# jovoy/SolarAxionRayTracing

Hardware: AMD Instinct MI355X
Metric: rays/sec (higher is better)
Workload: dtype f64

## Files before the change

### solaraxionraytracing_amd/csrc/sart_api.hip

```cpp
#include <hip/hip_runtime.h>
#include <rccl/rccl.h>
#include <dlfcn.h>
#include <sys/mman.h>
#include <unistd.h>

#include <algorithm>
#include <atomic>
#include <cmath>
#include <condition_variable>
#include <thread>
#include <cstdio>
#include <cstdlib>
#include <cstring>
#include <limits>
#include <map>
#include <mutex>
#include <string>
#include <vector>

#include "../../include/sart.h"
#include "sart_device.h"

namespace sart {
void launch_trace_histogram(const HotA& H, const HotB& HB, const DevBlob* blob, const TraceArgs& A, double* acc, int n_blocks,
// ... 16 lines not shown
                               double* shared_row, int n_blocks, hipStream_t stream, bool fast, bool fixed);
int angular_scan_blocks_per_cu(bool fast);
void launch_ascan_images(const HotA& H, const HotB& HB, const DevBlob* blob, const TraceArgs& A, const AScanArgs& AN, double* img_partials,
                         double* rows, double* shared_row, int n_blocks, hipStream_t stream, bool fast, bool fixed);
int ascan_images_blocks_per_cu(bool fast);
int energy_scan_blocks_per_cu(bool rotated);
void launch_trace_energy_scan(const HotA& H, const HotB& HB, const DevBlob* blob, const TraceArgs& A, const EScanArgs& EN, double* rows,
                              double* shared_row, int n_blocks, hipStream_t stream, bool rotated, bool fixed);
int shell_histogram_blocks_per_cu(bool rotated);
void launch_shell_histogram(const HotA& H, const HotB& HB, const DevBlob* blob, const TraceArgs& A, double* acc, const ShellArgs& SH,
                            int n_blocks, hipStream_t stream, bool rotated, bool fixed);
void launch_finalize_shells(const void* in, double* out, int n_shells, int n_energies1, int spectra, double q_w, double q_w2,
                            void* check_dev, hipStream_t stream);
int channel_histogram_blocks_per_cu(bool rotated);
void launch_channel_histogram(const HotA& H, const HotB& HB, const DevBlob* blob, const TraceArgs& A, double* acc, const ChannelArgs& CH,
                              int n_blocks, hipStream_t stream, bool rotated, bool fixed);
void launch_finalize_channels(const void* in, double* out, int n_channels, int n_energies1, int spectra, size_t n_img, double q_w,
                              double q_w2, void* check_dev, hipStream_t stream);
void launch_channel_fractions(const double* rates_dev, const double* total_dev, double* frac_dev, int n_channels, int stride,
                              size_t n_cells, unsigned long long* first_bad_dev, hipStream_t stream);
int origin_histogram_blocks_per_cu(bool rotated);
void launch_origin_histogram(const HotA& H, const HotB& HB, const DevBlob* blob, const TraceArgs& A, double* acc, const OriginArgs& OG,
                             int n_blocks, hipStream_t stream, bool rotated, bool fixed);
void launch_finalize_origin(const void* in, double* out, size_t n_cells, double q_w, double q_w2, void* check_dev, hipStream_t stream);
int aperture_histogram_blocks_per_cu(bool rotated);
void launch_aperture_histogram(const HotA& H, const HotB& HB, const DevBlob* blob, const TraceArgs& A, double* acc, const ApertureArgs& AP,
                               int n_blocks, hipStream_t stream, bool rotated, bool fixed);
int histogram_block_of(int variant);
void launch_trace_records(const HotA& H, const HotB& HB, const DevBlob* blob, const TraceArgs& A, sart_axion_t* out, int n_blocks,
                          hipStream_t stream, const double* uniforms_dev);
void launch_mirror_miss_count(const HotA& H, const DevBlob* blob, const TraceArgs& A, unsigned long long* counts, int n_blocks, hipStream_t stream);
void launch_radial_verdicts(const HotA& H, const DevBlob* blob, const double* radii, int n, uint32_t* out_table, uint32_t* out_compares,
                            hipStream_t stream);
int records_block();
int compact_chunk_max();
void launch_compact_records(const sart_axion_t* rec, uint32_t n, sart_axion_t* out, unsigned long long capacity, uint32_t* block_counts,
                            unsigned long long* block_first, unsigned long long* counts, hipStream_t stream);
void launch_stage_columns(const HotA& H, const HotB& HB, const DevBlob* blob, const TraceArgs& A, uint64_t* stage, uint32_t* flags,
                          uint32_t mask, int n_blocks, hipStream_t stream);
void launch_compact_columns(const uint64_t* stage, const uint32_t* flags, uint32_t n, uint32_t mask, unsigned long long ray_id0, uint64_t* out,
                            unsigned long long capacity, uint32_t* block_counts, unsigned long long* block_first,
                            unsigned long long* counts, hipStream_t stream);
int histogram_blocks_per_cu(int variant);
void launch_build_solar_tables(const double* em_dev, const double* radii_dev, const double* energies_dev, int n_radii, int n_energies,
                               double* cdf_dev, double* row_sum_dev, double* rcdf_dev, uint16_t* rguide_dev, uint16_t* eguide_dev,
                               uint32_t* status_dev, hipStream_t stream);
void launch_cdf_hi32(const double* cdf_dev, uint32_t* out_dev, size_t n, hipStream_t stream);
}

using namespace sart;

namespace {

thread_local std::string g_err;
int fail(int code, const std::string& msg) {
  g_err = msg;
  return code;
}
#define SART_HIP(call)                                                                              \
  do {                                                                                              \
    hipError_t e_ = (call);                                                                         \
    if (e_ != hipSuccess)                                                                           \
      return fail(e_ == hipErrorOutOfMemory ? SART_ERR_OUT_OF_MEMORY : SART_ERR_NO_DEVICE,          \
                  std::string(#call) + ": " + hipGetErrorString(e_));                               \
  } while (0)

// ... 1421 lines not shown
}

int sart_get_radial_table(sart_context* c, double* breakpoints, uint32_t* verdicts, uint8_t* cells, int32_t* n_cells) {
  if (!c) return fail(SART_ERR_INVALID_ARGUMENT, "ctx is NULL");
  SART_HIP(hipSetDevice(c->device));
  if (int rc = refresh_derived(c)) return rc;
  if (int rc = sync_blob(c)) return rc;
  if (n_cells) *n_cells = c->params.lut_n;
  if (c->radial_n > 0) {
    const uint8_t* t = c->shell_lut.data() + kRadialTableOffset;
    if (breakpoints) std::memcpy(breakpoints, t + offsetof(RadialLds, b), static_cast<size_t>(c->radial_n) * sizeof(double));
    if (verdicts) std::memcpy(verdicts, t + offsetof(RadialLds, w), static_cast<size_t>(c->radial_n) * sizeof(uint32_t));
    if (cells) std::memcpy(cells, c->shell_lut.data() + kRadialCellsOffset, static_cast<size_t>(c->params.lut_n));
  }
  return c->radial_n;
}

__attribute__((visibility("default"))) int sart_internal_radial_verdicts(sart_context* c, const double* radii, int32_t n, uint32_t* by_table,
                                                                         uint32_t* by_compares) {
  if (!c || !radii || !by_table || !by_compares || n < 1) return fail(SART_ERR_INVALID_ARGUMENT, "invalid argument");
  SART_HIP(hipSetDevice(c->device));
  if (int rc = refresh_derived(c)) return rc;
  if (int rc = sync_blob(c)) return rc;
  if (!c->hot.radial_table) return fail(SART_ERR_UNSUPPORTED, "this setup has no radial verdict table");
  DevBuf<double> d_r;
  DevBuf<uint32_t> d_out;
  if (int rc = d_r.upload(radii, static_cast<size_t>(n))) return rc;
  if (int rc = d_out.resize(2 * static_cast<size_t>(n))) return rc;
  launch_radial_verdicts(c->hot, c->d_blob.p, d_r.p, n, d_out.p, d_out.p + n, c->stream);
  SART_HIP(hipGetLastError());
  SART_HIP(hipMemcpyAsync(by_table, d_out.p, static_cast<size_t>(n) * sizeof(uint32_t), hipMemcpyDeviceToHost, c->stream));
  SART_HIP(hipMemcpyAsync(by_compares, d_out.p + n, static_cast<size_t>(n) * sizeof(uint32_t), hipMemcpyDeviceToHost, c->stream));
  SART_HIP(hipStreamSynchronize(c->stream));
  return 0;
}

namespace {

class HostPrefault {
 public:
  HostPrefault(char* base, size_t bytes, size_t chunk_bytes, bool enabled, unsigned threads, bool keep = false)
      : base_(base), bytes_(bytes), chunk_(chunk_bytes), threads_(threads ? threads : 8u), keep_(keep) {
    n_chunks_ = (bytes + chunk_bytes - 1) / chunk_bytes;
    if (!enabled || bytes < (size_t(8) << 20)) { done_ = n_chunks_; return; }
    const long page = sysconf(_SC_PAGESIZE);
    page_ = page > 0 ? static_cast<size_t>(page) : 4096;
    const uintptr_t lo = (reinterpret_cast<uintptr_t>(base) + page_ - 1) / page_ * page_;
    const uintptr_t hi = (reinterpret_cast<uintptr_t>(base) + bytes) / page_ * page_;
    if (hi > lo) (void)madvise(reinterpret_cast<void*>(lo), hi - lo, MADV_HUGEPAGE);
    worker_ = std::thread([this] { run(); });
  }
  ~HostPrefault() {
    allow(0, true);
    if (worker_.joinable()) worker_.join();
  }
  void wait(size_t k) {
    allow(k + 1);
    std::unique_lock<std::mutex> lock(m_);
    cv_.wait(lock, [&] { return done_ > k; });
  }
  void set_lazy() { std::lock_guard<std::mutex> lock(m_); allowed_ = 0; }
  void allow(size_t chunks, bool stop = false) {
    {
      std::lock_guard<std::mutex> lock(m_);
      allowed_ = std::max(allowed_, std::min(chunks, n_chunks_));
      stop_ = stop_ || stop;
// ... 1859 lines not shown
```

### solaraxionraytracing_amd/csrc/sart_kernels.hip

```cpp
#include <hip/hip_runtime.h>
#include <stdint.h>
#include <string.h>

#include <type_traits>

#include "../../include/sart.h"
#include "sart_device.h"
#include "sart_math.h"

namespace sart {

struct U4 { uint32_t x, y, z, w; };
constexpr int kPhiloxRounds = 7;

__device__ __forceinline__ U4 philox4x32(uint32_t c0, uint32_t c1, uint32_t c2, uint32_t c3, uint32_t k0,
                                         uint32_t k1) {
#pragma unroll
  for (int r = 0; r < kPhiloxRounds; ++r) {
    const uint64_t p0 = (uint64_t)0xD2511F53u * c0;
    const uint64_t p1 = (uint64_t)0xCD9E8D57u * c2;
    const uint32_t hi0 = (uint32_t)(p0 >> 32), lo0 = (uint32_t)p0;
    const uint32_t hi1 = (uint32_t)(p1 >> 32), lo1 = (uint32_t)p1;
    const uint32_t n0 = __builtin_amdgcn_bitop3_b32(hi1, c1, k0, 0x96);
    const uint32_t n2 = __builtin_amdgcn_bitop3_b32(hi0, c3, k1, 0x96);
// ... 1136 lines not shown
#ifndef SART_PRIO_B
#define SART_PRIO_B 3
#endif
#ifndef SART_PRIO_ACC
#define SART_PRIO_ACC 1
#endif
constexpr int kQueue = 128;

struct __align__(16) TablesLds {
  double sincos[2 * kSinCosEntries];
  uint32_t rcdf_hi[kMaxRadii + 4];
  ShellDev shells[kMaxShells];
  uint16_t rguide[kRadiusGuideEntries + 6];
  uint8_t lut[kShellLutMax];
};

struct __align__(16) WaveRings {
  double X0[kQueue], Y0[kQueue], tsx[kQueue], tsy[kQueue];
  double path[kQueue], u5[kQueue];
  int idx[kQueue];
  uint32_t ray[kQueue];
  uint32_t u3hi[kQueue];
};
struct __align__(16) HistRings {
  double X0[kQueue], Y0[kQueue], tsx[kQueue], tsy[kQueue];
  double path[kQueue];
  uint2 cell[kQueue];
  uint32_t ray[kQueue];
  uint32_t u3hi[kQueue];
};
static_assert(sizeof(WaveRings) - sizeof(HistRings) == kQueue * sizeof(uint32_t) && sizeof(HistRings) % 512 == 0 &&
                  (kTileRingCells / kQueue * (sizeof(WaveRings) - sizeof(HistRings))) / sizeof(double) == kTileExtraCells + kRadialTableCells - kRingExtraCells,
              "what ring 1's packed cell frees is what the histogram kernels' image tile grows by");
template <int WAVES, typename Rings = WaveRings>
struct __align__(16) QueueLds {
  Rings w[WAVES];
};

template <int BLOCK>
__device__ __forceinline__ void stage_tables(TablesLds& S, const DevParams& P, const DevTables& T, bool radial_cells = false) {
  for (int i = threadIdx.x; i < 2 * kSinCosEntries; i += BLOCK) S.sincos[i] = as_global(T.sincos_tab)[i];
  for (int i = threadIdx.x; i < P.n_radii + 4; i += BLOCK) {
    const double c = (i < P.n_radii) ? as_global(T.flux_radius_cdf)[i] : 1.0;
    const unsigned long long t = __double2ull_rd(c * 4503599627370496.0) >> 20;
    S.rcdf_hi[i] = t > 0xFFFFFFFFull ? 0xFFFFFFFFu : (uint32_t)t;
  }
  for (int i = threadIdx.x; i < kRadiusGuideEntries; i += BLOCK) S.rguide[i] = as_global(T.radius_guide)[i];
  {
    const auto src = as_global(reinterpret_cast<const uint64_t*>(T.shells));
    uint64_t* dst = reinterpret_cast<uint64_t*>(S.shells);
    const int n = P.n_shells * (int)(sizeof(ShellDev) / 8);
    for (int i = threadIdx.x; i < n; i += BLOCK) dst[i] = src[i];
  }
  const uint8_t* lut = T.shell_lut + (radial_cells ? kRadialCellsOffset : 0);
  for (int i = threadIdx.x; i < P.lut_n; i += BLOCK) S.lut[i] = as_global(lut)[i];
  __syncthreads();
}

__device__ __forceinline__ void reload_hot(HotA& dst) {
  typedef const __attribute__((address_space(4))) uint32_t* kernarg_ptr;
  kernarg_ptr p = (kernarg_ptr)__builtin_amdgcn_kernarg_segment_ptr();
  asm volatile("" : "+s"(p));
  uint32_t* d = reinterpret_cast<uint32_t*>(&dst);
#pragma unroll
  for (int k = 0; k < (int)(sizeof(HotA) / 4); ++k) d[k] = p[k];
}

struct ZoneTable {
  int32_t n_zones;
  uint32_t zone_reached;
  uint32_t lo[kMaxZones], hi[kMaxZones];
};
static_assert(sizeof(ZoneTable) == sizeof(HotA) - offsetof(HotA, n_zones), "ZoneTable mirrors the tail of HotA");
static_assert(offsetof(WaveRings, u3hi) == offsetof(WaveRings, ray) + kQueue * sizeof(uint32_t) && offsetof(WaveRings, ray) % 8 == 0 &&
                  offsetof(HistRings, u3hi) == offsetof(HistRings, ray) + kQueue * sizeof(uint32_t) && offsetof(HistRings, ray) % 8 == 0,
              "the image tile uses ray + u3hi of every wave as 128 contiguous doubles");
__device__ __forceinline__ void reload_zones(ZoneTable& dst) {
  typedef const __attribute__((address_space(4))) uint32_t* kernarg_ptr;
  kernarg_ptr p = (kernarg_ptr)__builtin_amdgcn_kernarg_segment_ptr() + offsetof(HotA, n_zones) / 4;
  asm volatile("" : "+s"(p));
  uint32_t* d = reinterpret_cast<uint32_t*>(&dst);
#pragma unroll
  for (int k = 0; k < (int)(sizeof(ZoneTable) / 4); ++k) d[k] = p[k];
}

struct HistKernArgs {
  HotA H;
  const DevBlob* blob;
  TraceArgs A;
  double* acc;
  HotB HB;
  ScanArgs SC;
};
static_assert(offsetof(HistKernArgs, H) == 0 && offsetof(HistKernArgs, blob) == (sizeof(HotA) + 7) / 8 * 8 &&
                  offsetof(HistKernArgs, A) == offsetof(HistKernArgs, blob) + 8 &&
                  offsetof(HistKernArgs, acc) == offsetof(HistKernArgs, A) + sizeof(TraceArgs) &&
                  offsetof(HistKernArgs, HB) == offsetof(HistKernArgs, acc) + 8 &&
                  offsetof(HistKernArgs, SC) == offsetof(HistKernArgs, HB) + sizeof(HotB) && sizeof(HotA) % 4 == 0 &&
                  sizeof(TraceArgs) % 8 == 0 && sizeof(HotB) % 8 == 0,
              "reload_hot / reload_zones / reload_kernarg read the arguments at these offsets");
template <typename T>
__device__ __forceinline__ void reload_kernarg(T& dst, size_t byte_offset) {
  static_assert(sizeof(T) % 4 == 0, "dword granularity");
  typedef const __attribute__((address_space(4))) uint32_t* kernarg_ptr;
  kernarg_ptr p = (kernarg_ptr)__builtin_amdgcn_kernarg_segment_ptr() + byte_offset / 4;
  asm volatile("" : "+s"(p));
  uint32_t* d = reinterpret_cast<uint32_t*>(&dst);
#pragma unroll
  for (int k = 0; k < (int)(sizeof(T) / 4); ++k) d[k] = p[k];
}

template <int BLOCK, bool FAST, bool ROT, int GAS, bool PATHC, bool FIXED, bool SCAN = false>
__global__ __launch_bounds__(BLOCK) void trace_histogram_kernel(HotA H, const DevBlob* __restrict__ blob, TraceArgs A,
                                                                double* __restrict__ acc, HotB HBarg, ScanArgs SCarg) {
  constexpr bool BANDS = false;
#include "sart_trace_histogram.inc"
// ... 2260 lines not shown
__global__ __launch_bounds__(256) void radial_verdict_kernel(HotA H, const DevBlob* __restrict__ blob, const double* __restrict__ radii, int n,
                                                             uint32_t* __restrict__ out_table, uint32_t* __restrict__ out_compares) {
  struct Lds {
    TablesLds S;
    RadialLds R;
    double behind[kRadialMarked + 1 - kRadialMax];
    DevBlob B;
  };
  __shared__ Lds lds;
  {
    const uint64_t* src = reinterpret_cast<const uint64_t*>(blob);
    uint64_t* dst = reinterpret_cast<uint64_t*>(&lds.B);
    for (int i = threadIdx.x; i < (int)(sizeof(DevBlob) / 8); i += 256) dst[i] = src[i];
    for (int i = threadIdx.x; i < kRadialMarked + 1 - kRadialMax; i += 256) lds.behind[i] = 0.0;
    __syncthreads();
  }
  const DevParams& P = lds.B.P;
  {
    const auto src = as_global(reinterpret_cast<const uint64_t*>(lds.B.T.shell_lut + kRadialTableOffset));
    uint64_t* dst = reinterpret_cast<uint64_t*>(&lds.R);
    for (int i = threadIdx.x; i < kRadialTableCells; i += 256) dst[i] = src[i];
  }
  stage_tables<256>(lds.S, P, lds.B.T, true);
  const LdsTables L{lds.S.sincos, lds.S.rcdf_hi, lds.B.T.flux_radius_cdf, lds.S.rguide, lds.S.shells, lds.S.lut, &lds.R, &lds.B.T};
  const bool cand_on = H.telescope_kind != SART_TK_LLNL;
  const int i = blockIdx.x * 256 + threadIdx.x;
  if (i < n) {
    const double radial = radii[i];
    out_table[i] = radial_verdict_table(H, P, L, cand_on, radial);
    out_compares[i] = radial_verdict_compares(H, P, L.shells, lds.B.T.shell_lut, cand_on, radial);
  }
}

__global__ __launch_bounds__(kRecBlock) void mirror_miss_count_kernel(HotA H, const DevBlob* __restrict__ blob, TraceArgs A,
                                                                       unsigned long long* __restrict__ counts) {
  __shared__ TablesLds S;
  __shared__ DevBlob B;
  {
    const uint64_t* src = reinterpret_cast<const uint64_t*>(blob);
    uint64_t* dst = reinterpret_cast<uint64_t*>(&B);
    for (int i = threadIdx.x; i < (int)(sizeof(DevBlob) / 8); i += kRecBlock) dst[i] = src[i];
    __syncthreads();
  }
  const DevParams& P = B.P;
  stage_tables<kRecBlock>(S, P, B.T);
  const LdsTables L{S.sincos, S.rcdf_hi, B.T.flux_radius_cdf, S.rguide, S.shells, S.lut};
  uint32_t n[5] = {0, 0, 0, 0, 0};
  const uint64_t stride = (uint64_t)gridDim.x * kRecBlock;
  const uint64_t n_round = (A.n_rays + stride - 1) / stride * stride;
  for (uint64_t i = (uint64_t)blockIdx.x * kRecBlock + threadIdx.x; i < n_round; i += stride) {
    RayState st;
    bool sampled, reached;
    double radial;
    LaneMasks masks;
    double r3sq;
    const uint64_t ray_id = A.ray_id_offset + i;
    const uint32_t u3_hi = word_of(stream_block(ray_id >> 2, A.seed_lo, A.seed_hi), (uint32_t)ray_id & 3u);
    const bool alive = phase_a<false, -1, false, false, false>(H, P, L, A.seed_lo, A.seed_hi, ray_id, u3_hi, st, sampled, reached, radial, masks, nullptr, &r3sq) &&
                       i < A.n_rays;
    const ShellDev& sh = L.shells[st.shell];
    const double X0 = st.X0, Y0 = st.Y0, tsx = st.tsx, tsy = st.tsy;
    const double Q0 = fma(X0, X0, Y0 * Y0), D0 = fma(X0, tsx, Y0 * tsy), A0 = fma(tsx, tsx, tsy * tsy);
    double z1;
    uint64_t hit1_m;
    const bool hit1 = pick_root(A0 - sh.m1_k, D0 + sh.m1_hb, Q0 - sh.m1_cc, 0.0, sh.m1_zhi, z1, hit1_m);
    const double zcb = st.zcb;
// ... 611 lines not shown
  for (int k = 0; k < n_masses; ++k) { F.q_w[k] = q_w[k]; F.q_w2[k] = q_w2[k]; }
  hipLaunchKernelGGL(finalize_scan_kernel, dim3(1), dim3(64), 0, stream, reinterpret_cast<const long long*>(in), out, F, static_cast<FixedCheck*>(check_dev));
}
void launch_finalize_scan_bands(const void* rows, const void* shared_row, const void* in, double* out, const void* counts_in, double* counts_out,
                                int n_masses, int n_cells, const double* q_w, const double* q_w2, void* check_dev, hipStream_t stream) {
  FinalizeBandsArgs F;
  memset(&F, 0, sizeof F);
  F.n_masses = n_masses;
  F.n_cells = n_cells;
  for (int k = 0; k < n_masses; ++k) { F.q_w[k] = q_w[k]; F.q_w2[k] = q_w2[k]; }
  hipLaunchKernelGGL(finalize_scan_bands_kernel, dim3(n_masses + (counts_in ? 1 : 0)), dim3(64), 0, stream, static_cast<const long long*>(rows),
                     static_cast<const long long*>(shared_row), static_cast<const long long*>(in), out, static_cast<const long long*>(counts_in),
                     counts_out, F, static_cast<FixedCheck*>(check_dev));
}
int compact_chunk_max() { return kCompactBlock * kCompactMaxBlocks; }
void launch_compact_records(const sart_axion_t* rec, uint32_t n, sart_axion_t* out, unsigned long long capacity, uint32_t* block_counts,
                            unsigned long long* block_first, unsigned long long* counts, hipStream_t stream) {
  const uint32_t n_blocks = (n + kCompactBlock - 1) / kCompactBlock;
  hipLaunchKernelGGL(records_count_kernel, dim3(n_blocks), dim3(kCompactBlock), 0, stream, rec, n, block_counts, counts);
  hipLaunchKernelGGL(records_scan_kernel, dim3(1), dim3(kCompactMaxBlocks), 0, stream, block_counts, n_blocks, block_first, counts, n);
  hipLaunchKernelGGL(records_scatter_kernel, dim3(n_blocks), dim3(kCompactBlock), 0, stream, rec, n, block_first, out, capacity);
}
void launch_trace_records(const HotA& H, const HotB& HB, const DevBlob* blob, const TraceArgs& A, sart_axion_t* out, int n_blocks,
                          hipStream_t stream, const double* uniforms_dev) {
  hipLaunchKernelGGL(trace_records_kernel, dim3(n_blocks), dim3(kRecBlock), 0, stream, H, blob, A, out, HB, uniforms_dev);
}
void launch_mirror_miss_count(const HotA& H, const DevBlob* blob, const TraceArgs& A, unsigned long long* counts, int n_blocks, hipStream_t stream) {
  hipLaunchKernelGGL(mirror_miss_count_kernel, dim3(n_blocks), dim3(kRecBlock), 0, stream, H, blob, A, counts);
}
void launch_radial_verdicts(const HotA& H, const DevBlob* blob, const double* radii, int n, uint32_t* out_table, uint32_t* out_compares,
                            hipStream_t stream) {
  hipLaunchKernelGGL(radial_verdict_kernel, dim3((n + 255) / 256), dim3(256), 0, stream, H, blob, radii, n, out_table, out_compares);
}
void launch_stage_columns(const HotA& H, const HotB& HB, const DevBlob* blob, const TraceArgs& A, uint64_t* stage, uint32_t* flags,
                          uint32_t mask, int n_blocks, hipStream_t stream) {
  hipLaunchKernelGGL(columns_stage_kernel, dim3(n_blocks), dim3(kRecBlock), 0, stream, H, blob, A, stage, flags, HB, mask);
}
void launch_compact_columns(const uint64_t* stage, const uint32_t* flags, uint32_t n, uint32_t mask, unsigned long long ray_id0, uint64_t* out,
                            unsigned long long capacity, uint32_t* block_counts, unsigned long long* block_first,
                            unsigned long long* counts, hipStream_t stream) {
  const uint32_t n_blocks = (n + kCompactBlock - 1) / kCompactBlock;
  hipLaunchKernelGGL(columns_count_kernel, dim3(n_blocks), dim3(kCompactBlock), 0, stream, flags, n, block_counts, counts);
  hipLaunchKernelGGL(records_scan_kernel, dim3(1), dim3(kCompactMaxBlocks), 0, stream, block_counts, n_blocks, block_first, counts, n);
  hipLaunchKernelGGL(columns_scatter_kernel, dim3(n_blocks), dim3(kCompactBlock), 0, stream, stage, flags, n, block_first, out, capacity, mask,
                     ray_id0);
}

}
```

### solaraxionraytracing_amd/csrc/sart_trace_histogram.inc

```
  struct LdsLayout {
    TablesLds S;
    RadialLds R;
    double tile_extra[kTileExtraCells];
    DevBlob B;
    TraceArgs Ab;
    QueueLds<BLOCK / 64, HistRings> Q;
  };
  static_assert(sizeof(RadialLds) % 8 == 0 && (kRadialMarked + 1) * sizeof(double) <= sizeof(RadialLds) + kTileExtraCells * sizeof(double),
                "entry kRadialMarked of either column lies in the table or in the tile's cells");
  __shared__ LdsLayout lds;
  TablesLds& S = lds.S;
  QueueLds<BLOCK / 64, HistRings>& Q = lds.Q;
  static_assert(!PATHC || (FAST && !ROT && GAS >= 0), "the constant-path form belongs to the unrotated specialisations");
  static_assert(!SCAN || GAS != 0, "a mass scan needs the gas stage");
  static_assert(!SCAN || kScanMaxMasses * 2 * kScanLanes <= (BLOCK / 64) * kQueue, "the scan accumulators live in the image tile's 128 doubles per wave");
  __shared__ uint32_t scan_zero[kScanMaxMasses];
  static_assert(!BANDS || SCAN, "the bands belong to the mass scan");
  __shared__ uint32_t scan_band_n[BANDS ? kScanLanes : 1];
  static_assert((BLOCK / 64) * kQueue == kTileRingCells && kImageTileMax * kImageTileMax <= kTileRingCells + kTileExtraCells &&
                    kImageTileExtraMax * kImageTileExtraMax <= kTileExtraCells && BLOCK / 64 == kTileRingCells / kQueue,
                "the LDS image tile (host: kImageTileMax): 128 doubles per wave of this workgroup's rings + the cells behind the tables");
  static_assert((offsetof(LdsLayout, Q) % 512) == 0, "the rings are addressed with ds_*2st64 offsets (units of 512 bytes for 64-bit columns)");
  auto tile_cell_lo = [&](uint32_t t) -> double* {
    return PATHC ? &Q.w[t >> 7].path[t & 127u] : reinterpret_cast<double*>(&Q.w[t >> 7].ray[0]) + (t & 127u);
  };
  auto tile_cell = [&](uint32_t t) -> double* {
    return t < (uint32_t)kTileRingCells ? tile_cell_lo(t) : &lds.tile_extra[t - (uint32_t)kTileRingCells];
  };
  DevBlob& B = lds.B;
  TraceArgs& Ab = lds.Ab;
  {
    const uint64_t* src = reinterpret_cast<const uint64_t*>(blob);
    uint64_t* dst = reinterpret_cast<uint64_t*>(&B);
    for (int i = threadIdx.x; i < (int)(sizeof(DevBlob) / 8); i += BLOCK) dst[i] = src[i];
    if (threadIdx.x == 0) Ab = A;
    __syncthreads();
  }
  const DevParams& Pb = B.P;
  const DevTables& Tb = B.T;
  {
    uint64_t* q = reinterpret_cast<uint64_t*>(&Q);
    for (int i = threadIdx.x; i < (int)(sizeof(Q) / 8); i += BLOCK) q[i] = 0ull;
    for (int i = threadIdx.x; i < kTileExtraCells; i += BLOCK) lds.tile_extra[i] = 0.0;
    if (SCAN && threadIdx.x < kScanMaxMasses) scan_zero[threadIdx.x] = 0u;
    if (BANDS && threadIdx.x < kScanLanes) scan_band_n[threadIdx.x] = 0u;
  }
  constexpr bool RTAB = FAST;
  if (RTAB && H.radial_table) {
    const auto src = as_global(reinterpret_cast<const uint64_t*>(Tb.shell_lut + kRadialTableOffset));
    uint64_t* dst = reinterpret_cast<uint64_t*>(&lds.R);
    for (int i = threadIdx.x; i < kRadialTableCells; i += BLOCK) dst[i] = src[i];
  }
  stage_tables<BLOCK>(S, Pb, Tb, RTAB && H.radial_table);
  const LdsTables L{S.sincos, S.rcdf_hi, Tb.flux_radius_cdf, S.rguide, S.shells, S.lut, &lds.R, &Tb};

  const int lane = threadIdx.x & 63;
  const int wave = __builtin_amdgcn_readfirstlane((int)(threadIdx.x >> 6));
  const uint64_t waves_total = (uint64_t)gridDim.x * (BLOCK / 64);
  const uint64_t wave_global = (uint64_t)blockIdx.x * (BLOCK / 64) + wave;
  const bool early_reject = (SCAN && !PATHC) ? false : H.n_zones > 0;
  const uint64_t first_chunk = A.ray_id_offset >> 8;
  uint64_t id_base = first_chunk << 8;
  asm volatile("" : "+s"(id_base));
  const uint32_t rel_begin = (uint32_t)(A.ray_id_offset & 255u);
  const uint32_t rel_end = rel_begin + (uint32_t)A.n_rays;
  const uint32_t n_chunks = (rel_end + 255u) >> 8;

  uint32_t n_reached = 0, n_shell = 0, n_nickel = 0, n_till = 0, n_passed = 0;
  uint32_t n_outside = 0;
  using Sum = std::conditional_t<FIXED, long long, double>;
  Sum sum_w = 0, sum_w2 = 0, sum_x = 0, sum_y = 0, sum_r = 0;
  long long sum_wo = 0;
#ifdef SART_STAGE_TIMING
  uint64_t cyc_a0 = 0, cyc_a1 = 0, cyc_b = 0, cyc_bs[6] = {0, 0, 0, 0, 0, 0};
#endif
  uint32_t h0 = 0, t0 = 0;
// ... 21 lines not shown
    HotA Hl;
    reload_hot(Hl);
    constexpr bool ZEXT = FAST && !ROT && GAS >= 0;
    LaneMasks M;
    double r3sq = 0.0;
    (void)phase_a<FAST, ROT ? 1 : 0, ZEXT, PATHC, true, RTAB>(Hl, Pb, L, A.seed_lo, A.seed_hi, id_base + (uint64_t)rel, u3_hi, st, sampled, reached, radial,
                                                              M, HOLD_SINCOS ? &Ksc : nullptr, ROT ? nullptr : &r3sq);
    const uint64_t valid_m = ballot64(valid);
    n_reached += (uint32_t)__popcll(valid_m & M.reached);
    const uint64_t selected = valid_m & M.ok;
    n_shell += (uint32_t)__popcll(selected);
    uint64_t sure = 0ull;
    const uint64_t cand = (ROT || Hl.telescope_kind == SART_TK_LLNL) ? 0ull
                                                                     : (selected & (RTAB ? M.cand : ballot64(radial > (double)Pb.mirror_miss_radius)));
    if (cand) {
      if (RTAB && Hl.radial_table) r3sq = L.shells[st.shell].n1_r3sq;
      const double zl = Pb.l_mirror, xe = fma(zl, st.tsx, st.X0), ye = fma(zl, st.tsy, st.Y0);
      sure = cand & ballot64(fma(xe, xe, fma(ye, ye, kMirrorMissEps)) < r3sq) &
             ballot64(fma(st.tsx, st.tsx, st.tsy * st.tsy) < (double)Pb.mirror_miss_slope_sq);
      n_nickel += (uint32_t)__popcll(sure);
    }
#ifdef SART_DEBUG_KNOBS
    const uint64_t mask = (A.flags & 0x10000000u) ? 0ull : (selected & (RTAB ? M.keep : ~ballot64(radial < Pb.shell0_miss_radius)) & ~sure);
#else
    const uint64_t mask = selected & (RTAB ? M.keep : ~ballot64(radial < Pb.shell0_miss_radius)) & ~sure;
#endif
    const bool alive = __builtin_amdgcn_inverse_ballot_w64(mask);
    const uint32_t cnt = (uint32_t)__popcll(mask);
    if (alive) {
      asm volatile("; hot: ring 1 write");
      const uint32_t slot = prefix_from(mask, t1) % kQueue;
      Q.w[wave].X0[slot] = st.X0; Q.w[wave].Y0[slot] = st.Y0;
      Q.w[wave].tsx[slot] = st.tsx; Q.w[wave].tsy[slot] = st.tsy;
      if (!PATHC) Q.w[wave].path[slot] = st.path_cb;
      Q.w[wave].cell[slot] = make_uint2((uint32_t)(st.r_idx | (st.shell << 16)), st.u5_hi);
    }
    t1 += cnt;
    __builtin_amdgcn_s_setprio(0);
  };

  auto run_phase_b = [&](uint32_t n_valid) {
    SART_STAGE_MARK("B");
    __builtin_amdgcn_s_setprio(SART_PRIO_B);
    RayState st;
    const bool valid = (uint32_t)lane < n_valid;
    const uint32_t slot = (h1 + (uint32_t)lane) % kQueue;
    RayOut out;
    {
      st.X0 = Q.w[wave].X0[slot]; st.Y0 = Q.w[wave].Y0[slot];
      st.tsx = Q.w[wave].tsx[slot]; st.tsy = Q.w[wave].tsy[slot];
      st.path_cb = PATHC ? H.length_b : Q.w[wave].path[slot];
      const uint2 cell = Q.w[wave].cell[slot];
      st.u5 = u52(cell.y, 0u);
      st.u5_hi = cell.y;
      if (!ROT) {
        st.zcb = -(H.dz3 - H.dz1);
      } else {
        st.zcb = zcb_rotated(Pb.rx_s, -Pb.rx_c * Pb.ry_s, Pb.rx_c * Pb.ry_c, Pb.half_length_telescope, st.X0 + Pb.entrance_x,
                             st.Y0 + Pb.entrance_y, st.tsx, st.tsy, H.dz3 - H.dz1);
      }
      const int packed = (int)cell.x;
      st.r_idx = packed & 0xFFFF;
      st.shell = packed >> 16;
      const DevBlob& Bo = lds_opaque(B);
      HotB HB;
      reload_kernarg(HB, offsetof(HistKernArgs, HB));
      asm volatile("" :: "s"(HB.cdf_hi32), "s"(HB.energy_guide), "s"(HB.energy_tab), "s"(HB.refl), "s"(HB.refl_n_angles), "s"(HB.cdf_stride));
      phase_b<false, FAST, GAS, FAST && !ROT && GAS >= 0, SCAN>(Bo.P, L, HB, lds_opaque(Ab), st, (!FAST && H.test_active) ? Pb.n_energies : -1, valid, out, nullptr);
      if constexpr (SCAN) {
        SART_STAGE_MARK("SCAN");
        n_passed += (uint32_t)__popcll(out.m_passed);
        struct { int32_t n_masses, pad; } hdr;
        reload_kernarg(hdr, offsetof(HistKernArgs, SC));
        const uint32_t fl = (uint32_t)__builtin_amdgcn_readfirstlane((int)Ab.flags);
        const bool use_prob = !(fl & SART_CF_IGNORE_CONV_PROB) & ((GAS >= 0) ? (GAS == 1) : (__builtin_amdgcn_readfirstlane(Bo.P.stage_gas) != 0));
        const double term1 = Bo.P.gas_term1;
        const GasCos cos_lead = GasCos::make();
        uint32_t cell = 0u;
        if constexpr (BANDS) {
          struct { int32_t e0; uint32_t mul; } b0;
          struct { uint32_t window, unused; } b1;
          reload_kernarg(b0, offsetof(HistKernArgs, SC) + offsetof(ScanArgs, m) + offsetof(ScanMass, aux));
          reload_kernarg(b1, offsetof(HistKernArgs, SC) + offsetof(ScanArgs, m) + sizeof(ScanMass) + offsetof(ScanMass, aux));
          const uint32_t d = (uint32_t)(out.e_idx - b0.e0);
// ... 61 lines not shown
        sum_w2 = fma(out.weight, out.weight, sum_w2);
        sum_x += out.px;
        sum_y += out.py;
        sum_r += out.rdet;
      }
      const double fx = (out.px - Al.image_x_min) * Al.image_inv_step_x;
      const double fy = (out.py - Al.image_y_min) * Al.image_inv_step_y;
      const int nx = Al.image_nx, ny = Al.image_ny;
      const uint64_t inside_m = ballot64(fx >= 0.0) & ballot64(fx < (double)nx) & ballot64(fy >= 0.0) & ballot64(fy < (double)ny);
      const bool inside = __builtin_amdgcn_inverse_ballot_w64(inside_m);
      n_outside += inside ? 0u : 1u;
      if constexpr (FIXED) {
        if (out.m_passed & ~inside_m) {
          asm volatile("; rare: passed rays outside the image");
          sum_wo += inside ? 0ll : w_fx;
        }
      }
#ifdef SART_DEBUG_KNOBS
      const uint32_t rep_key = (Al.flags & 0x08000000u) ? blockIdx.x : (uint32_t)wave_global;
      double* const img = Al.replicas + (size_t)(rep_key & Al.replica_mask) * (size_t)Al.replica_stride;
#else
      double* const img = Al.replicas + (size_t)((uint32_t)wave_global & Al.replica_mask) * (size_t)Al.replica_stride;
#endif
#ifdef SART_DEBUG_KNOBS
      if (inside && !(Al.flags & 0x40000000u))
#else
      if (inside)
#endif
      {
        const uint32_t ix = (uint32_t)(int)fx, iy = (uint32_t)(int)fy;
        const uint32_t tn = (uint32_t)Al.tile_n;
        const uint32_t tx = ix - (uint32_t)Al.tile_x0, ty = iy - (uint32_t)Al.tile_y0;
        if ((tx < tn) & (ty < tn)) {
          const uint32_t t = ty * tn + tx + (uint32_t)Al.tile_base;
          if constexpr (FIXED)
            __hip_atomic_fetch_add(reinterpret_cast<unsigned long long*>(tile_cell(t)), (unsigned long long)w_fx, __ATOMIC_RELAXED,
                                   __HIP_MEMORY_SCOPE_WORKGROUP);
          else
            __hip_atomic_fetch_add(tile_cell(t), out.weight, __ATOMIC_RELAXED, __HIP_MEMORY_SCOPE_WORKGROUP);
        } else {
          const uint32_t pix = iy * (uint32_t)nx + ix;
          typedef __attribute__((address_space(1))) char* gbytes;
          if constexpr (FIXED) atomic_add_slot_i64((double*)((gbytes)img + pix * 8u), w_fx);
          else unsafeAtomicAdd((double*)((gbytes)img + pix * 8u), out.weight);
        }
      }
      if (Al.spectra) {
        double* rad = acc + (size_t)nx * (size_t)ny + SART_ACC_COUNT;
        double* en = rad + 2 * (size_t)Al.n_radial_bins;
        const size_t ne1 = (size_t)Pb.n_energies + 1;
        const int rb = min((int)(out.rdet * Al.radial_inv_bin), Al.n_radial_bins - 1);
        if constexpr (FIXED) {
          atomic_add_slot_i64(&rad[rb], 1);
          atomic_add_slot_i64(&rad[(size_t)Al.n_radial_bins + rb], w_fx);
          atomic_add_slot_i64(&en[out.e_idx], 1);
          atomic_add_slot_i64(&en[ne1 + out.e_idx], w_fx);
          atomic_add_slot_i64(&en[2 * ne1 + out.e_idx], to_fixed(out.reflect, kFixedReflectScale));
        } else {
          unsafeAtomicAdd(&rad[rb], 1.0);
          unsafeAtomicAdd(&rad[(size_t)Al.n_radial_bins + rb], out.weight);
          unsafeAtomicAdd(&en[out.e_idx], 1.0);
          unsafeAtomicAdd(&en[ne1 + out.e_idx], out.weight);
          unsafeAtomicAdd(&en[2 * ne1 + out.e_idx], out.reflect);
        }
      }
    }
    __builtin_amdgcn_s_setprio(0);
  };

  constexpr bool kZonesInVgprs = FAST;
  uint32_t zone_lo_v[kMaxZones], zone_hi_v[kMaxZones];
#pragma unroll
  for (int z = 0; z < kMaxZones; ++z) {
    zone_lo_v[z] = H.zone_lo[z];
    zone_hi_v[z] = H.zone_hi[z];
    if (kZonesInVgprs) asm volatile("" : "+v"(zone_lo_v[z]), "+v"(zone_hi_v[z]));
  }
  uint32_t zone_reached_v = H.zone_reached;
  if (kZonesInVgprs) asm volatile("" : "+v"(zone_reached_v));
  uint32_t chunk = (uint32_t)wave_global;
  const uint32_t lane4 = 4u * (uint32_t)lane;
  uint32_t pass = 0;
  U4 stream = U4{0u, 0u, 0u, 0u};
#ifdef SART_STAGE_TIMING
  const uint64_t cyc_start = __builtin_readcyclecounter();
  const uint64_t real_start = __builtin_amdgcn_s_memrealtime();
#define SART_STAMP(var) const uint64_t var = __builtin_readcyclecounter()
#define SART_SPAN(acc, t_begin) acc += __builtin_readcyclecounter() - (t_begin)
#else
#define SART_STAMP(var)
#define SART_SPAN(acc, t_begin)
#endif
  for (;;) {
    const bool have_new = chunk < n_chunks;
    SART_STAGE_MARK("LOOP");
    if (have_new) {
      SART_STAGE_MARK("A0");
      SART_STAMP(ts_a0);
      if (pass == 0u) {
        asm volatile("; hot x0.25: one block of the shared word stream per four passes");
        stream = stream_block(((first_chunk + (uint64_t)chunk) << 6) + (uint64_t)lane, A.seed_lo, A.seed_hi);
      }
      const uint32_t w = stream.x;
      stream.x = stream.y; stream.y = stream.z; stream.z = stream.w;
      const uint32_t rel = ((chunk << 8) + pass) + lane4;
      if (early_reject) {
        ZoneTable Z;
        if constexpr (!kZonesInVgprs) reload_zones(Z);
        const uint32_t zone_reached = kZonesInVgprs ? (uint32_t)__builtin_amdgcn_readfirstlane((int)zone_reached_v) : Z.zone_reached;
        struct WordMasks { uint64_t mask, reached; };
        auto a0_masks = [&](uint32_t ww, uint32_t rr, uint32_t zr, uint32_t ck) -> WordMasks {
          uint64_t dead_m = 0, in_first = 0;
#pragma unroll
          for (int z = 0; z < kMaxZones; ++z) {
            const uint64_t in = kZonesInVgprs ? (ballot64(ww >= zone_lo_v[z]) & ballot64(ww <= zone_hi_v[z]))
                                              : (ballot64(ww >= Z.lo[z]) & ballot64(ww <= Z.hi[z]));
            dead_m |= in;
            if (z == 0) in_first = in;
          }
          const uint64_t reached_m = dead_m & ~((zr & 1u) ? 0ull : in_first);
          uint64_t valid_m = ~0ull;
          if (ck - 1u >= n_chunks - 2u) valid_m = ballot64(rr >= rel_begin) & ballot64(rr < rel_end);
#ifdef SART_DEBUG_KNOBS
          const uint64_t mask = (A.flags & 0x20000000u) ? 0ull : (valid_m & ~dead_m);
#else
          const uint64_t mask = valid_m & ~dead_m;
#endif
          return WordMasks{mask, valid_m & reached_m};
        };
        auto ring0_push = [&](uint64_t mask, uint32_t ww, uint32_t rr) {
          if (__builtin_amdgcn_inverse_ballot_w64(mask)) {
            asm volatile("; hot: ring 0 write");
            const uint32_t slot = prefix_from(mask, t0) % kQueue;
            Q.w[wave].ray[slot] = rr;
            Q.w[wave].u3hi[slot] = ww;
          }
          t0 += (uint32_t)__popcll(mask);
        };
        const WordMasks wa = a0_masks(w, rel, zone_reached, chunk);
        n_reached += (uint32_t)__popcll(wa.reached);
        ring0_push(wa.mask, w, rel);
        if ((zone_reached >> (pass + (uint32_t)kA0WideBit)) & 1u) {
          uint32_t zr = zone_reached, ck = chunk;
          asm volatile("" : "+s"(zr), "+s"(ck));
          const uint32_t wb = stream.x;
          const WordMasks mb = a0_masks(wb, rel + 1u, zr, ck);
          if ((t0 - h0) + (uint32_t)__popcll(mb.mask) <= (uint32_t)kQueue) {
            n_reached += (uint32_t)__popcll(mb.reached);
            ring0_push(mb.mask, wb, rel + 1u);
            stream.x = stream.y; stream.y = stream.z; stream.z = stream.w;
            pass += 1u;
          }
        }
      } else {
        run_phase_a(rel, (rel >= rel_begin) & (rel < rel_end), w);
      }
      pass = (pass + 1u) & 3u;
      if (pass == 0u) chunk += (uint32_t)waves_total;
      ring_sync();
      SART_SPAN(cyc_a0, ts_a0);
    }
// ... 37 lines not shown
      if (t1 == h1) break;
    }
  }

  SART_STAGE_MARK("EPILOGUE");
  if constexpr (SCAN) {
    __syncthreads();
    static_assert(2 * kScanLanes == 64, "one cell per lane");
    for (int k = wave; k < SCarg.n_masses; k += BLOCK / 64) {
      using Sum = std::conditional_t<FIXED, long long, double>;
      Sum* const dst = reinterpret_cast<Sum*>(SCarg.partials) + ((size_t)blockIdx.x * kScanMaxMasses + (size_t)k) * kScanPartialSlots;
      const double cell = *tile_cell_lo((uint32_t)k * 64u + (uint32_t)lane);
      Sum v;
      if constexpr (FIXED) v = __double_as_longlong(cell); else v = cell;
      if constexpr (BANDS)
        (reinterpret_cast<Sum*>(SCarg.partials) + (size_t)gridDim.x * (kScanMaxMasses * kScanPartialSlots))[(size_t)blockIdx.x * kScanBandSlots + (size_t)k * 64u + (size_t)lane] = v;
#pragma unroll
      for (int off = 16; off > 0; off >>= 1) v += __shfl_xor(v, off, 64);
      if (lane == 0) { dst[0] = v; dst[2] = (Sum)scan_zero[k]; dst[3] = 0; }
      if (lane == 32) dst[1] = v;
    }
    if constexpr (BANDS) {
      using Sum = std::conditional_t<FIXED, long long, double>;
      if (threadIdx.x < kScanLanes)
        (reinterpret_cast<Sum*>(SCarg.partials) + (size_t)gridDim.x * (kScanMaxMasses * kScanPartialSlots))[(size_t)blockIdx.x * kScanBandSlots + kScanMaxMasses * 64u + threadIdx.x] =
            (Sum)scan_band_n[threadIdx.x];
    }
  }
  if (!SCAN && A.tile_n > 0) {
    __syncthreads();
    const uint32_t tn = (uint32_t)A.tile_n, n_tile = tn * tn;
    double* const img = A.replicas + (size_t)((uint32_t)wave_global & A.replica_mask) * (size_t)A.replica_stride;
    for (uint32_t t = threadIdx.x; t < n_tile; t += BLOCK) {
      const double v = *tile_cell(t + (uint32_t)A.tile_base);
      if (__double_as_longlong(v) != 0ll) {
        const uint32_t ty = t / tn, tx = t - ty * tn;
        double* const px = &img[(size_t)((uint32_t)A.tile_y0 + ty) * (size_t)A.image_nx + ((uint32_t)A.tile_x0 + tx)];
        if constexpr (FIXED) atomic_add_slot_i64(px, __double_as_longlong(v));
        else unsafeAtomicAdd(px, v);
      }
    }
  }

  static_assert(sizeof(Sum) * (BLOCK / 64) * SART_ACC_COUNT <= 3 * kQueue * sizeof(double) && offsetof(HistRings, Y0) == kQueue * sizeof(double) &&
                    offsetof(HistRings, tsx) == 2 * kQueue * sizeof(double), "the scalar staging area fits the first three ring columns of wave 0");
  __syncthreads();
  Sum (*const red)[SART_ACC_COUNT] = reinterpret_cast<Sum (*)[SART_ACC_COUNT]>(&Q.w[0].X0[0]);
  Sum sw, sw2, sxx, syy, srr;
  if constexpr (FIXED) {
    sw = wave_sum_i64(sum_w); sw2 = wave_sum_i64(sum_w2); sxx = wave_sum_i64(sum_x); syy = wave_sum_i64(sum_y); srr = wave_sum_i64(sum_r);
  } else {
    sw = wave_sum(sum_w); sw2 = wave_sum(sum_w2); sxx = wave_sum(sum_x); syy = wave_sum(sum_y); srr = wave_sum(sum_r);
  }
  const long long swo = FIXED ? wave_sum_i64(sum_wo) : 0ll;
  const long long n_out = wave_sum_i64((long long)n_outside);
  if (lane == 0) {
    Sum* r = red[wave];
    for (int k = 0; k < SART_ACC_COUNT; ++k) r[k] = 0;
    r[SART_ACC_SUM_WEIGHTS] = sw;
    r[SART_ACC_SUM_WEIGHTS_SQ] = sw2;
    r[SART_ACC_SUM_X] = sxx;
    r[SART_ACC_SUM_Y] = syy;
    r[SART_ACC_SUM_R] = srr;
    r[SART_ACC_N_PASSED] = (Sum)n_passed;
    r[SART_ACC_N_PASSED_TILL_WINDOW] = (Sum)n_till;
    r[SART_ACC_N_HIT_NICKEL] = (Sum)n_nickel;
    r[SART_ACC_N_REACHED_TELESCOPE] = (Sum)n_reached;
    r[SART_ACC_N_SHELL_SELECTED] = (Sum)n_shell;
    r[SART_ACC_N_OUTSIDE_IMAGE] = (Sum)n_out;
    if constexpr (FIXED) r[SART_ACC_SUM_WEIGHTS_OUTSIDE] = swo;
#ifdef SART_STAGE_TIMING
    r[12] = (Sum)cyc_a0; r[13] = (Sum)cyc_a1; r[14] = (Sum)cyc_b;
    r[15] = (Sum)(__builtin_readcyclecounter() - cyc_start);
    r[SART_ACC_N_HIT_NICKEL] = (Sum)(__builtin_amdgcn_s_memrealtime() - real_start);
    r[SART_ACC_SUM_X] = (Sum)cyc_bs[0]; r[SART_ACC_SUM_Y] = (Sum)cyc_bs[1]; r[SART_ACC_SUM_R] = (Sum)cyc_bs[2];
    r[SART_ACC_SUM_WEIGHTS_SQ] = (Sum)cyc_bs[3]; r[SART_ACC_N_OUTSIDE_IMAGE] = (Sum)cyc_bs[4];
#endif
  }
// ... 7 lines not shown
```

Measured before the change: 111.7 billion.

## Use contiguous LDS image tile and single-compare zone test in stage A0

```diff
diff --git a/solaraxionraytracing_amd/csrc/sart_api.hip b/solaraxionraytracing_amd/csrc/sart_api.hip
--- a/solaraxionraytracing_amd/csrc/sart_api.hip
+++ b/solaraxionraytracing_amd/csrc/sart_api.hip
@@ -72,6 +72,7 @@
 void launch_mirror_miss_count(const HotA& H, const DevBlob* blob, const TraceArgs& A, unsigned long long* counts, int n_blocks, hipStream_t stream);
 void launch_radial_verdicts(const HotA& H, const DevBlob* blob, const double* radii, int n, uint32_t* out_table, uint32_t* out_compares,
                             hipStream_t stream);
+void launch_a0_masks(const HotA& H, const uint32_t* words, int n, uint32_t* out, hipStream_t stream);
 int records_block();
 int compact_chunk_max();
 void launch_compact_records(const sart_axion_t* rec, uint32_t n, sart_axion_t* out, unsigned long long capacity, uint32_t* block_counts,
@@ -1559,6 +1560,28 @@
   SART_HIP(hipMemcpyAsync(by_table, d_out.p, static_cast<size_t>(n) * sizeof(uint32_t), hipMemcpyDeviceToHost, c->stream));
   SART_HIP(hipMemcpyAsync(by_compares, d_out.p + n, static_cast<size_t>(n) * sizeof(uint32_t), hipMemcpyDeviceToHost, c->stream));
   SART_HIP(hipStreamSynchronize(c->stream));
+  return 0;
+}
+
+__attribute__((visibility("default"))) int sart_internal_a0_masks(sart_context* c, const uint32_t* words, int32_t n, uint32_t* out) {
+  if (!c || !words || !out || n < 1) return fail(SART_ERR_INVALID_ARGUMENT, "invalid argument");
+  SART_HIP(hipSetDevice(c->device));
+  if (int rc = refresh_derived(c)) return rc;
+  if (int rc = sync_blob(c)) return rc;
+  if (c->hot.n_zones < 1) return fail(SART_ERR_UNSUPPORTED, "this setup has no stage-A0 zones");
+  DevBuf<uint32_t> d_w, d_out;
+  if (int rc = d_w.upload(words, static_cast<size_t>(n))) return rc;
+  if (int rc = d_out.resize(static_cast<size_t>(n))) return rc;
+  launch_a0_masks(c->hot, d_w.p, n, d_out.p, c->stream);
+  SART_HIP(hipGetLastError());
+  SART_HIP(hipMemcpyAsync(out, d_out.p, static_cast<size_t>(n) * sizeof(uint32_t), hipMemcpyDeviceToHost, c->stream));
+  SART_HIP(hipStreamSynchronize(c->stream));
+  return 0;
+}
+
+__attribute__((visibility("default"))) int sart_internal_image_tile(sart_context* c, int32_t* out) {
+  if (!c || !out || !c->tile.valid) return -1;
+  out[0] = c->tile.x0; out[1] = c->tile.y0; out[2] = c->tile.n;
   return 0;
 }
 
diff --git a/solaraxionraytracing_amd/csrc/sart_kernels.hip b/solaraxionraytracing_amd/csrc/sart_kernels.hip
--- a/solaraxionraytracing_amd/csrc/sart_kernels.hip
+++ b/solaraxionraytracing_amd/csrc/sart_kernels.hip
@@ -1192,6 +1192,19 @@
 static_assert(sizeof(WaveRings) - sizeof(HistRings) == kQueue * sizeof(uint32_t) && sizeof(HistRings) % 512 == 0 &&
                   (kTileRingCells / kQueue * (sizeof(WaveRings) - sizeof(HistRings))) / sizeof(double) == kTileExtraCells + kRadialTableCells - kRingExtraCells,
               "what ring 1's packed cell frees is what the histogram kernels' image tile grows by");
+#ifndef SART_TILE_CONTIGUOUS
+#define SART_TILE_CONTIGUOUS 1
+#endif
+struct __align__(16) HistRingsConst {
+  double X0[kQueue], Y0[kQueue], tsx[kQueue], tsy[kQueue];
+  uint2 cell[kQueue];
+  uint32_t ray[kQueue];
+  uint32_t u3hi[kQueue];
+};
+static_assert(sizeof(HistRings) - sizeof(HistRingsConst) == kQueue * sizeof(double) && sizeof(HistRingsConst) % 512 == 0 &&
+                  (kTileRingCells / kQueue) * (sizeof(HistRings) - sizeof(HistRingsConst)) == kTileRingCells * sizeof(double) &&
+                  offsetof(HistRingsConst, cell) == offsetof(HistRings, path),
+              "the path column of 16 waves is what the contiguous tile holds beside the cells behind the tables");
 template <int WAVES, typename Rings = WaveRings>
 struct __align__(16) QueueLds {
   Rings w[WAVES];
@@ -1242,6 +1255,54 @@
   uint32_t* d = reinterpret_cast<uint32_t*>(&dst);
 #pragma unroll
   for (int k = 0; k < (int)(sizeof(ZoneTable) / 4); ++k) d[k] = p[k];
+}
+
+#ifndef SART_A0_ZONE_FORM
+#define SART_A0_ZONE_FORM 1
+#endif
+static_assert(SART_A0_ZONE_FORM >= 0 && SART_A0_ZONE_FORM <= 2, "SART_A0_ZONE_FORM: 0, 1 or 2");
+template <int FORM>
+__device__ __forceinline__ void a0_zone_operands(const HotA& H, uint32_t (&lo)[kMaxZones], uint32_t (&b)[kMaxZones]) {
+  uint32_t last_lo = H.zone_lo[0], last_hi = H.zone_hi[0];
+#pragma unroll
+  for (int z = 1; z < kMaxZones; ++z)
+    if (H.zone_lo[z] <= H.zone_hi[z]) { last_lo = H.zone_lo[z]; last_hi = H.zone_hi[z]; }
+#pragma unroll
+  for (int z = 0; z < kMaxZones; ++z) {
+    const bool empty = FORM != 0 && H.zone_lo[z] > H.zone_hi[z];
+    lo[z] = empty ? last_lo : H.zone_lo[z];
+    const uint32_t hi = empty ? last_hi : H.zone_hi[z];
+    b[z] = FORM != 0 ? hi - lo[z] : hi;
+  }
+}
+struct WordMasks { uint64_t mask, reached; };
+template <int FORM>
+__device__ __forceinline__ WordMasks a0_word_masks(uint32_t ww, uint32_t rr, uint32_t zr, uint32_t ck, const uint32_t (&lo)[kMaxZones],
+                                                   const uint32_t (&b)[kMaxZones], uint32_t n_chunks, uint32_t rel_begin, uint32_t rel_end,
+                                                   bool drop_all) {
+  uint64_t dead_m = 0, in_first = 0;
+  if constexpr (FORM == 2) {
+    uint32_t s[kMaxZones];
+#pragma unroll
+    for (int z = 0; z < kMaxZones; ++z) s[z] = __builtin_elementwise_sub_sat(ww - lo[z], b[z]);
+    uint32_t m = s[0];
+#pragma unroll
+    for (int z = 1; z < kMaxZones; ++z) m = min(m, s[z]);
+    dead_m = ballot64(m == 0u);
+    in_first = ballot64(s[0] == 0u);
+  } else {
+#pragma unroll
+    for (int z = 0; z < kMaxZones; ++z) {
+      const uint64_t in = FORM == 1 ? ballot64(ww - lo[z] <= b[z]) : (ballot64(ww >= lo[z]) & ballot64(ww <= b[z]));
+      dead_m |= in;
+      if (z == 0) in_first = in;
+    }
+  }
+  const uint64_t reached_m = dead_m & ~((zr & 1u) ? 0ull : in_first);
+  uint64_t valid_m = ~0ull;
+  if (ck - 1u >= n_chunks - 2u) valid_m = ballot64(rr >= rel_begin) & ballot64(rr < rel_end);
+  const uint64_t mask = drop_all ? 0ull : (valid_m & ~dead_m);
+  return WordMasks{mask, valid_m & reached_m};
 }
 
 struct HistKernArgs {
@@ -3568,6 +3629,17 @@
   }
 }
 
+__global__ __launch_bounds__(64) void a0_masks_kernel(HotA H, const uint32_t* __restrict__ words, int n, uint32_t* __restrict__ out) {
+  uint32_t lo[kMaxZones], b[kMaxZones];
+  a0_zone_operands<SART_A0_ZONE_FORM>(H, lo, b);
+#pragma unroll
+  for (int z = 0; z < kMaxZones; ++z) asm volatile("" : "+v"(lo[z]), "+v"(b[z]));
+  const int i = blockIdx.x * 64 + threadIdx.x;
+  const uint32_t w = i < n ? words[i] : 0u;
+  const WordMasks m = a0_word_masks<SART_A0_ZONE_FORM>(w, 0u, H.zone_reached, 1u, lo, b, 4u, 0u, 1u, false);
+  if (i < n) out[i] = (uint32_t)((m.mask >> threadIdx.x) & 1ull) | ((uint32_t)((m.reached >> threadIdx.x) & 1ull) << 1);
+}
+
 __global__ __launch_bounds__(kRecBlock) void mirror_miss_count_kernel(HotA H, const DevBlob* __restrict__ blob, TraceArgs A,
                                                                        unsigned long long* __restrict__ counts) {
   __shared__ TablesLds S;
@@ -4245,6 +4317,9 @@
                             hipStream_t stream) {
   hipLaunchKernelGGL(radial_verdict_kernel, dim3((n + 255) / 256), dim3(256), 0, stream, H, blob, radii, n, out_table, out_compares);
 }
+void launch_a0_masks(const HotA& H, const uint32_t* words, int n, uint32_t* out, hipStream_t stream) {
+  hipLaunchKernelGGL(a0_masks_kernel, dim3((n + 63) / 64), dim3(64), 0, stream, H, words, n, out);
+}
 void launch_stage_columns(const HotA& H, const HotB& HB, const DevBlob* blob, const TraceArgs& A, uint64_t* stage, uint32_t* flags,
                           uint32_t mask, int n_blocks, hipStream_t stream) {
   hipLaunchKernelGGL(columns_stage_kernel, dim3(n_blocks), dim3(kRecBlock), 0, stream, H, blob, A, stage, flags, HB, mask);
diff --git a/solaraxionraytracing_amd/csrc/sart_trace_histogram.inc b/solaraxionraytracing_amd/csrc/sart_trace_histogram.inc
--- a/solaraxionraytracing_amd/csrc/sart_trace_histogram.inc
+++ b/solaraxionraytracing_amd/csrc/sart_trace_histogram.inc
@@ -1,16 +1,31 @@
-  struct LdsLayout {
+  constexpr bool CTILE = PATHC && SART_TILE_CONTIGUOUS;
+  using Rings = std::conditional_t<CTILE, HistRingsConst, HistRings>;
+  constexpr int kTileArrayCells = kTileExtraCells + (CTILE ? kTileRingCells : 0);
+  struct LdsSplit {
     TablesLds S;
     RadialLds R;
-    double tile_extra[kTileExtraCells];
+    double tile[kTileExtraCells];
     DevBlob B;
     TraceArgs Ab;
     QueueLds<BLOCK / 64, HistRings> Q;
   };
-  static_assert(sizeof(RadialLds) % 8 == 0 && (kRadialMarked + 1) * sizeof(double) <= sizeof(RadialLds) + kTileExtraCells * sizeof(double),
-                "entry kRadialMarked of either column lies in the table or in the tile's cells");
+  struct LdsConst {
+    TablesLds S;
+    RadialLds R;
+    DevBlob B;
+    TraceArgs Ab;
+    char pad[(512 - (sizeof(TablesLds) + sizeof(RadialLds) + sizeof(DevBlob) + sizeof(TraceArgs)) % 512) % 512];
+    QueueLds<BLOCK / 64, HistRingsConst> Q;
+    double tile[kTileRingCells + kTileExtraCells];
+  };
+  using LdsLayout = std::conditional_t<CTILE, LdsConst, LdsSplit>;
+  static_assert(sizeof(RadialLds) % 8 == 0 && (kRadialMarked + 1) * sizeof(double) <= sizeof(RadialLds) + kTileExtraCells * sizeof(double) &&
+                    (kRadialMarked + 1) * sizeof(double) <= sizeof(RadialLds) + sizeof(DevBlob) &&
+                    sizeof(LdsLayout::tile) == kTileArrayCells * sizeof(double) && sizeof(LdsConst) <= sizeof(LdsSplit) + 512,
+                "entry kRadialMarked of either column lies in the table or in what follows it in this object");
   __shared__ LdsLayout lds;
   TablesLds& S = lds.S;
-  QueueLds<BLOCK / 64, HistRings>& Q = lds.Q;
+  QueueLds<BLOCK / 64, Rings>& Q = lds.Q;
   static_assert(!PATHC || (FAST && !ROT && GAS >= 0), "the constant-path form belongs to the unrotated specialisations");
   static_assert(!SCAN || GAS != 0, "a mass scan needs the gas stage");
   static_assert(!SCAN || kScanMaxMasses * 2 * kScanLanes <= (BLOCK / 64) * kQueue, "the scan accumulators live in the image tile's 128 doubles per wave");
@@ -20,12 +35,18 @@
   static_assert((BLOCK / 64) * kQueue == kTileRingCells && kImageTileMax * kImageTileMax <= kTileRingCells + kTileExtraCells &&
                     kImageTileExtraMax * kImageTileExtraMax <= kTileExtraCells && BLOCK / 64 == kTileRingCells / kQueue,
                 "the LDS image tile (host: kImageTileMax): 128 doubles per wave of this workgroup's rings + the cells behind the tables");
-  static_assert((offsetof(LdsLayout, Q) % 512) == 0, "the rings are addressed with ds_*2st64 offsets (units of 512 bytes for 64-bit columns)");
+  static_assert(!CTILE || (kImageTileMax * kImageTileMax <= kTileArrayCells && kScanMaxMasses * 2 * kScanLanes <= kTileArrayCells &&
+                           kTileArrayCells == kTileRingCells + kTileExtraCells),
+                "the contiguous tile holds the largest image tile the host hands a constant-path variant, and the scan's accumulators");
+  static_assert((offsetof(LdsLayout, Q) % 512) == 0 && sizeof(Rings) % 512 == 0,
+                "the rings are addressed with ds_*2st64 offsets (units of 512 bytes for 64-bit columns)");
   auto tile_cell_lo = [&](uint32_t t) -> double* {
-    return PATHC ? &Q.w[t >> 7].path[t & 127u] : reinterpret_cast<double*>(&Q.w[t >> 7].ray[0]) + (t & 127u);
+    if constexpr (CTILE) return &lds.tile[t];
+    else return PATHC ? &Q.w[t >> 7].path[t & 127u] : reinterpret_cast<double*>(&Q.w[t >> 7].ray[0]) + (t & 127u);
   };
   auto tile_cell = [&](uint32_t t) -> double* {
-    return t < (uint32_t)kTileRingCells ? tile_cell_lo(t) : &lds.tile_extra[t - (uint32_t)kTileRingCells];
+    if constexpr (CTILE) return &lds.tile[t];
+    else return t < (uint32_t)kTileRingCells ? tile_cell_lo(t) : &lds.tile[t - (uint32_t)kTileRingCells];
   };
   DevBlob& B = lds.B;
   TraceArgs& Ab = lds.Ab;
@@ -41,7 +62,7 @@
   {
     uint64_t* q = reinterpret_cast<uint64_t*>(&Q);
     for (int i = threadIdx.x; i < (int)(sizeof(Q) / 8); i += BLOCK) q[i] = 0ull;
-    for (int i = threadIdx.x; i < kTileExtraCells; i += BLOCK) lds.tile_extra[i] = 0.0;
+    for (int i = threadIdx.x; i < kTileArrayCells; i += BLOCK) lds.tile[i] = 0.0;
     if (SCAN && threadIdx.x < kScanMaxMasses) scan_zero[threadIdx.x] = 0u;
     if (BANDS && threadIdx.x < kScanLanes) scan_band_n[threadIdx.x] = 0u;
   }
@@ -129,7 +150,7 @@
       const uint32_t slot = prefix_from(mask, t1) % kQueue;
       Q.w[wave].X0[slot] = st.X0; Q.w[wave].Y0[slot] = st.Y0;
       Q.w[wave].tsx[slot] = st.tsx; Q.w[wave].tsy[slot] = st.tsy;
-      if (!PATHC) Q.w[wave].path[slot] = st.path_cb;
+      if constexpr (!PATHC) Q.w[wave].path[slot] = st.path_cb;
       Q.w[wave].cell[slot] = make_uint2((uint32_t)(st.r_idx | (st.shell << 16)), st.u5_hi);
     }
     t1 += cnt;
@@ -146,7 +167,8 @@
     {
       st.X0 = Q.w[wave].X0[slot]; st.Y0 = Q.w[wave].Y0[slot];
       st.tsx = Q.w[wave].tsx[slot]; st.tsy = Q.w[wave].tsy[slot];
-      st.path_cb = PATHC ? H.length_b : Q.w[wave].path[slot];
+      if constexpr (PATHC) st.path_cb = H.length_b;
+      else st.path_cb = Q.w[wave].path[slot];
       const uint2 cell = Q.w[wave].cell[slot];
       st.u5 = u52(cell.y, 0u);
       st.u5_hi = cell.y;
@@ -274,7 +296,7 @@
         const uint32_t tn = (uint32_t)Al.tile_n;
         const uint32_t tx = ix - (uint32_t)Al.tile_x0, ty = iy - (uint32_t)Al.tile_y0;
         if ((tx < tn) & (ty < tn)) {
-          const uint32_t t = ty * tn + tx + (uint32_t)Al.tile_base;
+          const uint32_t t = ty * tn + tx + (CTILE ? 0u : (uint32_t)Al.tile_base);
           if constexpr (FIXED)
             __hip_atomic_fetch_add(reinterpret_cast<unsigned long long*>(tile_cell(t)), (unsigned long long)w_fx, __ATOMIC_RELAXED,
                                    __HIP_MEMORY_SCOPE_WORKGROUP);
@@ -311,11 +333,11 @@
   };
 
   constexpr bool kZonesInVgprs = FAST;
+  constexpr int kZoneForm = kZonesInVgprs ? SART_A0_ZONE_FORM : 0;
   uint32_t zone_lo_v[kMaxZones], zone_hi_v[kMaxZones];
+  a0_zone_operands<kZoneForm>(H, zone_lo_v, zone_hi_v);
 #pragma unroll
   for (int z = 0; z < kMaxZones; ++z) {
-    zone_lo_v[z] = H.zone_lo[z];
-    zone_hi_v[z] = H.zone_hi[z];
     if (kZonesInVgprs) asm volatile("" : "+v"(zone_lo_v[z]), "+v"(zone_hi_v[z]));
   }
   uint32_t zone_reached_v = H.zone_reached;
@@ -350,25 +372,14 @@
         ZoneTable Z;
         if constexpr (!kZonesInVgprs) reload_zones(Z);
         const uint32_t zone_reached = kZonesInVgprs ? (uint32_t)__builtin_amdgcn_readfirstlane((int)zone_reached_v) : Z.zone_reached;
-        struct WordMasks { uint64_t mask, reached; };
         auto a0_masks = [&](uint32_t ww, uint32_t rr, uint32_t zr, uint32_t ck) -> WordMasks {
-          uint64_t dead_m = 0, in_first = 0;
-#pragma unroll
-          for (int z = 0; z < kMaxZones; ++z) {
-            const uint64_t in = kZonesInVgprs ? (ballot64(ww >= zone_lo_v[z]) & ballot64(ww <= zone_hi_v[z]))
-                                              : (ballot64(ww >= Z.lo[z]) & ballot64(ww <= Z.hi[z]));
-            dead_m |= in;
-            if (z == 0) in_first = in;
-          }
-          const uint64_t reached_m = dead_m & ~((zr & 1u) ? 0ull : in_first);
-          uint64_t valid_m = ~0ull;
-          if (ck - 1u >= n_chunks - 2u) valid_m = ballot64(rr >= rel_begin) & ballot64(rr < rel_end);
 #ifdef SART_DEBUG_KNOBS
-          const uint64_t mask = (A.flags & 0x20000000u) ? 0ull : (valid_m & ~dead_m);
+          const bool drop_all = (A.flags & 0x20000000u) != 0u;
 #else
-          const uint64_t mask = valid_m & ~dead_m;
-#endif
-          return WordMasks{mask, valid_m & reached_m};
+          constexpr bool drop_all = false;
+#endif
+          return a0_word_masks<kZoneForm>(ww, rr, zr, ck, kZonesInVgprs ? zone_lo_v : Z.lo, kZonesInVgprs ? zone_hi_v : Z.hi, n_chunks,
+                                          rel_begin, rel_end, drop_all);
         };
         auto ring0_push = [&](uint64_t mask, uint32_t ww, uint32_t rr) {
           if (__builtin_amdgcn_inverse_ballot_w64(mask)) {
@@ -472,7 +483,7 @@
     const uint32_t tn = (uint32_t)A.tile_n, n_tile = tn * tn;
     double* const img = A.replicas + (size_t)((uint32_t)wave_global & A.replica_mask) * (size_t)A.replica_stride;
     for (uint32_t t = threadIdx.x; t < n_tile; t += BLOCK) {
-      const double v = *tile_cell(t + (uint32_t)A.tile_base);
+      const double v = *tile_cell(t + (CTILE ? 0u : (uint32_t)A.tile_base));
       if (__double_as_longlong(v) != 0ll) {
         const uint32_t ty = t / tn, tx = t - ty * tn;
         double* const px = &img[(size_t)((uint32_t)A.tile_y0 + ty) * (size_t)A.image_nx + ((uint32_t)A.tile_x0 + tx)];
@@ -482,8 +493,9 @@
     }
   }
 
-  static_assert(sizeof(Sum) * (BLOCK / 64) * SART_ACC_COUNT <= 3 * kQueue * sizeof(double) && offsetof(HistRings, Y0) == kQueue * sizeof(double) &&
-                    offsetof(HistRings, tsx) == 2 * kQueue * sizeof(double), "the scalar staging area fits the first three ring columns of wave 0");
+  static_assert(sizeof(Sum) * (BLOCK / 64) * SART_ACC_COUNT <= 3 * kQueue * sizeof(double) && offsetof(Rings, Y0) == kQueue * sizeof(double) &&
+                    offsetof(Rings, tsx) == 2 * kQueue * sizeof(double) && offsetof(Rings, X0) == 0,
+                "the scalar staging area fits the first three ring columns of wave 0 (either ring layout)");
   __syncthreads();
   Sum (*const red)[SART_ACC_COUNT] = reinterpret_cast<Sum (*)[SART_ACC_COUNT]>(&Q.w[0].X0[0]);
   Sum sw, sw2, sxx, syy, srr;
```

Result: no change. 112.5 billion, median of 6 (+0.7%).
